# the-lay/voltools

Hardware: AMD Instinct MI355X
Metric: Mvoxels/s, 512^3 f32 filt_bspline StaticVolume transform (resident source, device output) (higher is better)
Workload: dtype f32; 1 GPU; 512^3 float32 filt_bspline, StaticVolume resident in HBM, rotate((0,i,0)) rzxz sweep, output= device buffer; lds_bytes=34816, kernel=8, resident_bytes=1660944384, angles=i

## Files before the change

voltools_amd/csrc/vt_api.hip:

```cpp
#include "vt_internal.h"
#include "vt_device.h"
#include "vt_host.h"

#include <atomic>
#include <cmath>
#include <cstdarg>
#include <cstdio>
#include <cstdlib>
#include <chrono>
#include <cstring>
#include <mutex>
#include <new>
#include <unordered_map>
#include <vector>

#include <unistd.h>

using namespace vt;

namespace vt_guard {
constexpr size_t kGuard = (size_t)1 << 20;
struct Entry { void* base; size_t bytes; };
static std::mutex mu;
static std::unordered_map<void*, Entry> live;
// ... 804 lines not shown
                VT_HIP(hipMalloc(&v->d_tplan, need));
                v->tplan_bytes = need;
                v->tplan_epoch = 0;
            }
            if (v->tplan_epoch == 0 || v->tplan_epoch == 0xffffffffu) {
                VT_HIP(hipMemsetAsync(v->d_tplan, 0, v->tplan_bytes, v->stream));
                v->tplan_epoch = 0;
            }
            q.tplan = v->d_tplan;
            q.tplan_epoch = ++v->tplan_epoch;
        }
        VT_HIP(launch_affine_quad(plan.cfg, v->interp, srcq, d_out, q, plan.grid, plan.lds_bytes, v->stream));
#ifdef VT_LEGACY
    } else if (plan.kind == 5) {
        float* const srcp = copy_ptr(v, kCopyP0 + ori.quad_idx);
        if (!srcp) return fail(VT_EINVAL, "internal: plane-pair copy missing");
        VT_HIP(launch_affine_zpair(plan.cfg, v->interp, srcp, d_out, p, plan.grid, plan.lds_bytes, v->stream));
#endif
    } else if (plan.kind == 9 || plan.kind == 6) {
        if (!v->d_queue) {
            VT_HIP(hipMalloc(reinterpret_cast<void**>(&v->d_queue), 9 * 128));
            VT_HIP(hipMemsetAsync(v->d_queue, 0, 9 * 128, v->stream));
        }
        if (plan.kind == 9) {
#ifdef VT_EXPERIMENTS
            static const int exp_lds = std::getenv("VT_EXP_BLOCK_LDS") ? std::atoi(std::getenv("VT_EXP_BLOCK_LDS")) : 0;
            static const int exp_grid = std::getenv("VT_EXP_BLOCK_GRID") ? std::atoi(std::getenv("VT_EXP_BLOCK_GRID")) : 0;
            VT_HIP(launch_affine_block(plan.cfg, plan.th, v->interp, ori.src_plain, d_out, v->d_zeros, v->d_queue, p, plan.geo, exp_grid > 0 ? exp_grid : plan.grid,
                                       std::max(plan.lds_bytes, exp_lds), v->stream));
#else
            VT_HIP(launch_affine_block(plan.cfg, plan.th, v->interp, ori.src_plain, d_out, v->d_zeros, v->d_queue, p, plan.geo, plan.grid, plan.lds_bytes, v->stream));
#endif
        }
        else if (!is_cubic(v->interp) && v->tune.span != 0)
            VT_HIP(launch_affine_span(plan.cfg, ori.src_plain, d_out, v->d_zeros, v->d_queue, p, plan.geo, plan.grid, plan.lds_bytes, v->stream));
        else
            VT_HIP(launch_affine_packed(plan.cfg, v->interp, ori.src_plain, d_out, v->d_zeros, v->d_queue, p, plan.geo, plan.grid, plan.lds_bytes, v->stream));
#ifdef VT_LEGACY
    } else if (plan.kind == 4) {
        VT_HIP(launch_affine_march(plan.cfg, v->interp, ori.src_plain, d_out, p, plan.grid, plan.lds_bytes, v->stream));
#endif
    } else if (plan.kind == 10) {
        VT_HIP(launch_affine_rows(v->interp, plan.td, ori.src_plain, d_out, v->d_zeros, p, plan.lds_bytes, v->stream));
    } else if (plan.kind >= 2) {
        VT_HIP(launch_affine_tiled(plan.cfg, v->interp, plan.kind == 3, ori.src_plain, d_out, v->d_zeros, p, plan.grid, plan.lds_bytes, v->stream));
    } else {
        VT_HIP(launch_affine_direct(v->interp, v->d_src, d_out, p, v->stream));
    }
    note_launch(v, plan.kind >= 2 ? plan.kind : 1, plan, p, n_out);
    return 0;
}

int host_output_buffer(vt_volume* v, size_t n_elems, float** d_out)
{
// ... 1484 lines not shown
                                (size_t)v->W * sizeof(float), rows, hipMemcpyDeviceToDevice, v->stream));
    else
        VT_HIP(pin.copy2d(v->d_src + (size_t)first_plane * v->H * v->P, (size_t)v->P * sizeof(float), data, (size_t)v->W * sizeof(float), rows, true, v->stream));
    VT_HIP(hipStreamSynchronize(v->stream));
    return 0;
}

int vt_volume_finalize(vt_volume_t* v)
{
    if (!v) return fail(VT_EINVAL, "NULL handle");
    if (!v->deferred) return 0;
    int rc = use_device(v->dev);
    if (rc) return rc;
    return finalize_resident(v, v->lo_interior);
}

int vt_volume_destroy(vt_volume_t* v)
{
    if (!v) return 0;
    hipSetDevice(v->dev);
    if (v->stream) hipStreamSynchronize(v->stream);
    if (v->d_src) cached_free(v->dev, v->d_src, v->src_bytes);
    if (v->d_queue) hipFree(v->d_queue);
    if (v->d_tplan) hipFree(v->d_tplan);
    {
        LazyCopies::Released rel;
        v->lazy.release_all(rel);
        for (void* b : rel.bufs) hipFree(b);
    }
    if (v->d_scratch_out) cached_free(v->dev, v->d_scratch_out, v->scratch_elems * sizeof(float));
    if (v->d_proj_tmp) hipFree(v->d_proj_tmp);
    if (v->d_proj_part) cached_free(v->dev, v->d_proj_part, v->proj_part_bytes);
    if (v->d_batch_m) hipFree(v->d_batch_m);
    if (v->proj) { vt_volume_destroy(v->proj); v->proj = nullptr; }
    if (v->ev0) recycle_event(v->dev, v->ev0);
    if (v->ev1) recycle_event(v->dev, v->ev1);
    if (v->evc0) (void)hipEventDestroy(v->evc0);
    if (v->evc1) (void)hipEventDestroy(v->evc1);
    if (v->stream && v->owns_stream) recycle_stream(v->dev, v->stream);
    delete v;
    return 0;
}

int vt_volume_release_copies(vt_volume_t* v, uint64_t* freed_bytes)
{
    if (!v) return fail(VT_EINVAL, "NULL argument");
// ... 314 lines not shown
```

voltools_amd/csrc/vt_device.h:

```cpp
#pragma once
#include "vt_internal.h"

namespace vt {


__host__ __device__ __forceinline__ void bspline_weights(float f, float& w0, float& w1, float& w2, float& w3)
{
    const float one_frac = 1.0f - f;
    const float squared = f * f;
    const float one_sqd = one_frac * one_frac;
    w0 = (1.0f / 6.0f) * one_sqd * one_frac;
    w1 = (2.0f / 3.0f) - 0.5f * squared * (2.0f - f);
    w2 = (2.0f / 3.0f) - 0.5f * one_sqd * (2.0f - one_frac);
    w3 = (1.0f / 6.0f) * squared * f;
}

__host__ __device__ __forceinline__ float bspline_fn(float t)
{
    t = fabsf(t);
    const float a = 2.0f - t;
    return (t < 1.0f) ? ((2.0f / 3.0f) - 0.5f * t * t * a) : ((t < 2.0f) ? (a * a * a * (1.0f / 6.0f)) : 0.0f);
}

template <bool SIMPLE>
// ... 12 lines not shown

__device__ __forceinline__ int wave_scan_add(int x)
{
    x += __builtin_amdgcn_update_dpp(0, x, 0x111, 0xf, 0xf, false);
    x += __builtin_amdgcn_update_dpp(0, x, 0x112, 0xf, 0xf, false);
    x += __builtin_amdgcn_update_dpp(0, x, 0x114, 0xf, 0xf, false);
    x += __builtin_amdgcn_update_dpp(0, x, 0x118, 0xf, 0xf, false);
    x += __builtin_amdgcn_update_dpp(0, x, 0x142, 0xa, 0xf, false);
    x += __builtin_amdgcn_update_dpp(0, x, 0x143, 0xc, 0xf, false);
    return x;
}
__device__ __forceinline__ int wave_scan_max(int x)
{
    x = max(x, __builtin_amdgcn_update_dpp(-1, x, 0x111, 0xf, 0xf, false));
    x = max(x, __builtin_amdgcn_update_dpp(-1, x, 0x112, 0xf, 0xf, false));
    x = max(x, __builtin_amdgcn_update_dpp(-1, x, 0x114, 0xf, 0xf, false));
    x = max(x, __builtin_amdgcn_update_dpp(-1, x, 0x118, 0xf, 0xf, false));
    x = max(x, __builtin_amdgcn_update_dpp(-1, x, 0x142, 0xa, 0xf, false));
    x = max(x, __builtin_amdgcn_update_dpp(-1, x, 0x143, 0xc, 0xf, false));
    return x;
}
__device__ __forceinline__ int wave_shift_up1(int x, int first) { return __builtin_amdgcn_update_dpp(first, x, 0x138, 0xf, 0xf, false); }

__device__ __forceinline__ int xcd_contiguous(int b, int n)
{
    const int xcd = b & 7, q = n >> 3, r = n & 7;
    const int start = (xcd < r) ? xcd * (q + 1) : r * (q + 1) + (xcd - r) * q;
    return start + (b >> 3);
}


__device__ __forceinline__ void march_tile(const AffineParams& p, int t, int& th_i, int& tw_i, int& chunk)
{
    const int per_layer = p.nTh * p.nTw;
    chunk = t / per_layer;
    const int u = t - chunk * per_layer;
    if (p.blk_h > 0) {
        const int col_tiles = p.nTh * p.blk_w;
        const int bc = u / col_tiles;
        const int wc = min(p.blk_w, p.nTw - bc * p.blk_w);
        const int u1 = u - bc * col_tiles;
        const int blk_tiles = p.blk_h * wc;
        const int br = u1 / blk_tiles;
        const int u2 = u1 - br * blk_tiles;
        const int r = u2 / wc;
        th_i = br * p.blk_h + r;
        tw_i = bc * p.blk_w + (u2 - r * wc);
    } else if (p.flags & (1 << 24)) {
        tw_i = u / p.nTh;
        th_i = u - tw_i * p.nTh;
    } else {
        th_i = u / p.nTw;
        tw_i = u - th_i * p.nTw;
    }
}

__host__ __device__ __forceinline__ int blocked_tile_count(int nTd, int nTh, int nTw)
{
    return ((nTd + 3) >> 2) * ((nTh + 3) >> 2) * ((nTw + 3) >> 2) * 64;
}
__device__ __forceinline__ bool blocked_tile(int t, int nTd, int nTh, int nTw, int& td, int& th, int& tw)
{
    const int nSh = (nTh + 3) >> 2, nSw = (nTw + 3) >> 2;
    const int sb = t >> 6, l = t & 63;
    const int sw = sb % nSw, s2 = sb / nSw;
    const int sh = s2 % nSh, sd = s2 / nSh;
    td = sd * 4 + (l >> 4);
    th = sh * 4 + ((l >> 2) & 3);
    tw = sw * 4 + (l & 3);
    return td < nTd && th < nTh && tw < nTw;
}

struct Fx { int hi; unsigned lo; };

constexpr double kBoxMargin = 0x1p-24;

__device__ __forceinline__ Fx to_fx(double x)
{
    const double fl = floor(x);
    Fx r;
    r.hi = (int)fl;
    r.lo = (unsigned)((x - fl) * 4294967296.0);
    return r;
}

__device__ __forceinline__ void fx_step(Fx& c, int inc_hi, unsigned inc_lo)
{
    const unsigned lo = c.lo + inc_lo;
    c.hi += inc_hi + (lo < c.lo ? 1 : 0);
    c.lo = lo;
}

__device__ __forceinline__ float fx_frac(const Fx& c) { return (float)c.lo * 0x1p-32f; }
// ... 189 lines not shown
```

voltools_amd/csrc/vt_host.h:

```cpp
#pragma once
#include "vt_internal.h"
#include "vt_resident.h"

#include <algorithm>
#include <cstdlib>
#include <vector>

struct Tuning {
    int tile = -1;
    int la = 0;
    int march_box = -1;
    int lxpad = -1;
    int dch = 0;
    int blk_h = -1, blk_w = -1;
    bool plain_tile_order = false;
    int rswap_wfast = -1;
    bool exp_nostore = false;
    bool exp_noload = false;
    bool exp_nolds = false;
    bool exp_noloop = false;
    bool exp_stamps = false;
    bool exp_notiles = false;
    bool exp_static = false;
    int quad_rows = -2;
// ... 2 lines not shown
    bool test_fail_copy = false;
    int quad_perm = 1;
    bool no_proj_cache = false;
    int quad_pingpong = 1;
    int quad_zid = 1;
    int reorient = 4;
    int rows_pd = 8;
    int no_fused_relayout = 0;
    int rows_db = 0;
    int rows = 1;
    int quad_zfir = 1;
    int zid_dch = 0;
    int quad_nt = -1;
    bool no_block = false;
    int block_rs = -1;
    bool block_linear = false;
    bool block_no_trim = false;
    int block_min = 240;
    int block_pad = -1;
    double max_resident_gb = 0.0;
    int span = 1;
    int span_pipe = 0;
    int block_th = 8;
    int64_t dot_part_cap = 64ll << 20;
    void read()
    {
        auto num = [](const char* name, int dflt) { const char* e = std::getenv(name); return e ? std::atoi(e) : dflt; };
        tile = num("VT_TILE", -1);
#ifdef VT_LEGACY
        la = num("VT_LA", 0);
        march_box = num("VT_MARCH_BOX", -1);
        if (march_box > 1) march_box = 1;
        lxpad = num("VT_LXPAD", -1);
#endif
        dch = std::max(0, num("VT_DCH", 0));
        blk_h = num("VT_BLK_H", -1);
        blk_w = num("VT_BLK_W", -1);
        plain_tile_order = num("VT_TILE_ORDER", 1) == 0;
        rswap_wfast = num("VT_RSWAP_WFAST", -1);
#ifdef VT_EXPERIMENTS
        exp_nostore = std::getenv("VT_EXP_NOSTORE") != nullptr;
        exp_noload = std::getenv("VT_EXP_NOLOAD") != nullptr;
        exp_nolds = std::getenv("VT_EXP_NOLDS") != nullptr;
        exp_noloop = std::getenv("VT_EXP_NOLOOP") != nullptr;
        exp_static = std::getenv("VT_EXP_STATIC") != nullptr;
        exp_notiles = std::getenv("VT_EXP_NOTILES") != nullptr;
// ... 2 lines not shown
        quad_nt = num("VT_QUAD_NT", -1);
#ifdef VT_LEGACY
        test_fail_copy = std::getenv("VT_TEST_FAIL_COPY") != nullptr;
        quad_perm = num("VT_QUAD_PERM", 1);
        quad_zid = num("VT_QUAD_ZID", 1);
        quad_grid2d = num("VT_QUAD_GRID2D", 1);
#endif
        quad_pingpong = num("VT_QUAD_PINGPONG", 1);
        quad_zfir = num("VT_QUAD_ZFIR", 1);
        rows = num("VT_ROWS", 1);
        rows_pd = num("VT_ROWS_PD", 8);
        rows_db = num("VT_ROWS_DB", 0);
        no_fused_relayout = num("VT_NO_FUSED_RELAYOUT", 0);
        reorient = num("VT_REORIENT", 4);
        no_proj_cache = std::getenv("VT_NO_PROJ_CACHE") != nullptr;
        zid_dch = num("VT_ZID_DCH", 0);
        quad_reverse = num("VT_QUAD_REVERSE", -1);
        quad_rows = num("VT_QUAD_ROWS", -2);
        no_block = std::getenv("VT_NO_BLOCK_KERNEL") != nullptr;
        block_rs = num("VT_BLOCK_RS", -1);
        block_linear = std::getenv("VT_BLOCK_LINEAR") != nullptr;
        block_pad = num("VT_BLOCK_PAD", -1);
        block_th = num("VT_BLOCK_TH", 8) == 16 ? 16 : 8;
        span_pipe = num("VT_SPAN_PIPE", 0);
        span = num("VT_SPAN", 1);
        { const char* e = std::getenv("VT_MAX_RESIDENT_GB"); max_resident_gb = e ? std::atof(e) : 0.0; }
        block_min = std::max(1, num("VT_BLOCK_MIN", 240));
        block_no_trim = std::getenv("VT_BLOCK_NO_TRIM") != nullptr;
        { const char* e = std::getenv("VT_DOT_PART_CAP"); if (e && std::atoll(e) > 0) dot_part_cap = std::min<int64_t>(std::atoll(e), 64ll << 20); }
    }
};


struct vt_volume {
    unsigned launch_no = 0;
    int dev = 0;
    int interp = 0;
    int D = 0, H = 0, W = 0;
    int oD = 0, oH = 0, oW = 0;
    int64_t plane0 = 0;
    int64_t gD = 0;
    int64_t out_plane0 = 0;
    int P = 0;
    float* d_src = nullptr;
    size_t src_bytes = 0;
    float* d_zeros = nullptr;
    int Pr = 0;
    int Px = 0;
    int reorient_asked[3] = {0, 0, 0};
    vt::LazyCopies lazy;
    float copies_ms = 0.f;
    int copies_built = 0, copies_evicted = 0;
    hipEvent_t evc0 = nullptr, evc1 = nullptr;
    int* d_queue = nullptr;
    void* d_tplan = nullptr;
    size_t tplan_bytes = 0;
    uint32_t tplan_epoch = 0;
    float* d_scratch_out = nullptr;
    double* d_batch_m = nullptr;
    std::vector<double> h_batch_m;
    size_t batch_m_cap = 0;
    float* d_proj_tmp = nullptr;
    size_t proj_tmp_elems = 0;
    double* d_proj_part = nullptr;
    size_t proj_part_bytes = 0;
    vt_volume* proj = nullptr;
    bool proj_sum_valid = false;
    double proj_sum_m3 = 0.0;
    int proj_sum_oD = 0;
    int64_t proj_sum_oplane0 = 0;
    int edge_pad = 0;
    bool stack = false;
    bool owns_stream = true;
    bool deferred = false;
    bool lo_interior = false;
    size_t scratch_elems = 0;
    hipStream_t stream = nullptr;
// ... 20 lines not shown
```

voltools_amd/csrc/vt_internal.h:

```cpp
#pragma once
#include <hip/hip_runtime.h>
#include <math.h>
#include <stdint.h>
#include "../../include/voltools_hip.h"

namespace vt {

constexpr float kPole   = -0x1.126148p-2f;
constexpr float kLambda =  0x1.7ffffep+2f;
constexpr float kAntiInit = 0x1.b0cb1ap-3f;

struct AffineParams {
    double m[12];
    double neg[3];
    double pos[3];
    double vlo[3];
    double vhi[3];
    int32_t inc_hi[3];
    uint32_t inc_lo[3];
    int32_t sD, sH, sW;
    int32_t sP;
    int32_t oD, oH, oW;
    int32_t nTd, nTh, nTw;
    int32_t Lz, Ly, Lx;
// ... 161 lines not shown
hipError_t launch_relayout_swap01(const float* src, float* dst, int D, int H, int P, hipStream_t stream);
int quad_max_it();
int quad_config_count();
void quad_config(int idx, int* th, int* tw, int* nt);
int quad_tile_plan_granules(int cfg);
int quad_tile_plan_lds(int cfg);
int quad_blocks_per_cu(int cfg, int interp, int lds_bytes, bool zid = false);
hipError_t init_quad_kernels();
hipError_t launch_relayout_zquad(const float* src, float* dst, int D, int H, int W, int P, int Pq, hipStream_t stream);
hipError_t launch_relayout_xfir(const float* src, float* dst, int D, int H, int W, int P, bool simple, hipStream_t stream);
hipError_t init_rows_kernels();
void rows_tile(int* ph, int* run);
hipError_t launch_affine_rows(int interp, int pd, const float* src, float* out, const float* zeros16, const AffineParams& p, int lds_bytes, hipStream_t stream);
hipError_t launch_relayout_zquad_fir(const float* src, float* dst, int D, int H, int W, int P, int Pq, bool simple, hipStream_t stream);
hipError_t launch_relayout_zquad_swap12(const float* src, float* dst, int D, int H, int W, int P, int Pq, bool fir, bool simple, hipStream_t stream);
hipError_t launch_affine_quad(int cfg, int interp, const float* srcq, float* out, const AffineParams& p,
                              int grid, int lds_bytes, hipStream_t stream);
int block_rs_count();
int block_rs(int idx);
int block_rs_order(int th, const int** order);
int block_max_vectors(int th);
void block_tile(int th, int* td, int* tw);
hipError_t init_block_kernels();
hipError_t launch_affine_block(int rs_idx, int th, int interp, const float* src, float* out, const float* zeros16, int* queue,
                               const AffineParams& p, const PackGeom& geo, int grid, int lds_bytes, hipStream_t stream);
int packed_config_count();
void packed_config(int idx, int* td, int* th, int* tw);
int packed_rows_max();
int packed_vectors_max();
hipError_t init_packed_kernels();
hipError_t launch_affine_packed(int cfg, int interp, const float* src, float* out, const float* zeros16, int* queue,
                                const AffineParams& p, const PackGeom& geo, int grid, int lds_bytes, hipStream_t stream);
int span_config_count();
void span_config(int idx, int* td, int* th, int* tw);
int span_rows_max();
bool span_config_pipelined(int idx);
int span_vectors_max();
hipError_t init_span_kernels();
hipError_t launch_affine_span(int cfg, const float* src, float* out, const float* zeros16, int* queue,
                              const AffineParams& p, const PackGeom& geo, int grid, int lds_bytes, hipStream_t stream);
int march_rows_max();
int march_max_it();
int interp_kind(int interp);
hipError_t init_march_kernels();
hipError_t launch_affine_march(int cfg, int interp, const float* src, float* out, const AffineParams& p,
                               int grid, int lds_bytes, hipStream_t stream);
hipError_t launch_affine_direct(int interp, const float* src, float* out, const AffineParams& p,
// ... 94 lines not shown
```

voltools_amd/csrc/vt_kernels_block.hip:

```cpp
#include "vt_internal.h"
#include "vt_device.h"

#include <algorithm>
#include <type_traits>

namespace vt {

typedef float v2f __attribute__((ext_vector_type(2)));

constexpr int kBlkTD = 8, kBlkTW = 16;
constexpr int block_max_it(int th) { return th == 16 ? 20 : 13; }

template <int OFF>
__device__ __forceinline__ void lds_read_b64(v2f& r, unsigned a)
{
    asm volatile("ds_read_b64 %0, %1 offset:%2" : "=v"(r) : "v"(a), "n"(OFF));
}

__device__ __forceinline__ v2f pk_fma(v2f a, float w, v2f c) { return __builtin_elementwise_fma(a, (v2f)(w), c); }

__device__ __forceinline__ void bspline_weights_pk(float f, v2f& w30, v2f& w12)
{
    const v2f fg = {f, 1.0f - f};
    const v2f sq = fg * fg;
// ... 66 lines not shown
                         (unsigned)gx < (unsigned)p.sP;
        const float* g = inb ? src + (((int64_t)gz * p.sH + gy) * p.sP + gx) : zeros16;
        __builtin_amdgcn_global_load_lds((const __attribute__((address_space(1))) void*)g,
                                         (__attribute__((address_space(3))) void*)(lds + 4 * vb), 16, 0, 0);
    }
}

template <int RS, int MAXIT>
__device__ __forceinline__ void stage_block_checked(float* lds, const float* __restrict__ src, const float* __restrict__ zeros16,
                                                    const AffineParams& p, const int (&o)[3], const int (&voff)[MAXIT], int total, int psv, int tid)
{
    constexpr int nvx = RS / 4;
    const int wave_first = __builtin_amdgcn_readfirstlane(tid & ~63);
    const char* const origin = reinterpret_cast<const char*>(src + (((int64_t)o[0] * p.sH + o[1]) * p.sP + o[2]));
#pragma unroll
    for (int k = 0; k < MAXIT; ++k) {
        if (k * 256 + wave_first < total) {
            int v = k * 256 + tid;
            asm volatile("" : "+v"(v));
            const int z = (int)__umulhi((unsigned)v, p.psv_magic), rem = v - z * psv;
            const int y = rem / nvx, cx = rem - y * nvx;
            const int gz = o[0] + z, gy = o[1] + y, gx = o[2] + 4 * cx;
            const bool inb = (unsigned)gz < (unsigned)p.sD && (unsigned)gy < (unsigned)p.sH && (unsigned)gx < (unsigned)p.sP;
            const float* g = inb ? reinterpret_cast<const float*>(origin + voff[k]) : zeros16;
            if (voff[k] != 0 || v == 0)
                __builtin_amdgcn_global_load_lds((const __attribute__((address_space(1))) void*)g,
                                                 (__attribute__((address_space(3))) void*)(lds + 4 * (k * 256 + wave_first)), 16, 0, 0);
        }
    }
}

template <int KIND, int RS, int TH>
__device__ __forceinline__ void affine_block_body(const float* __restrict__ src, float* __restrict__ out, const float* __restrict__ zeros16,
                                                  int* __restrict__ queue, const AffineParams& p, const PackGeom& geo)
{
    constexpr bool CUBIC = KIND != 0;
    constexpr int HALO = CUBIC ? 1 : 0;
    constexpr int TD = kBlkTD, TW = kBlkTW;
    constexpr int NS = TH == 16 ? 8 : 4;
    constexpr int kBlkMaxIt = block_max_it(TH);
    constexpr bool PIN = TH == 16;
    constexpr int nvx = RS / 4;
    extern __shared__ __attribute__((aligned(16))) float lds[];

    const int tid = threadIdx.x, lane = tid & 63, wv = tid >> 6;
    const int wave_first = __builtin_amdgcn_readfirstlane(tid & ~63);
    const int vd = lane >> 4, vh = 4 * (wv >> 1) + ((lane >> 2) & 3), vw = 4 * (wv & 1) + (lane & 3);
    constexpr int sd[8] = {0, 0, TH == 16 ? 0 : 4, TH == 16 ? 0 : 4, 4, 4, 4, 4};
    constexpr int sh[8] = {0, 0, TH == 16 ? 8 : 0, TH == 16 ? 8 : 0, 8, 8, 0, 0};
    constexpr int sw[8] = {0, 8, 8, 0, 0, 8, 8, 0};
    constexpr int which[7] = {0, TH == 16 ? 1 : 3, 2, 3, 0, 4, 2};

    const int Lz = p.Lz, Ly = p.Ly, ps = p.Lps;
    const int psv = ps >> 2;
    const int total = Lz * psv;
    const int nvx_used = p.Lx_used >> 2;
    const int row_b = p.sP * 4;
    const int plane_b = p.sH * row_b;

    int voff[kBlkMaxIt];
#pragma unroll
    for (int k = 0; k < kBlkMaxIt; ++k) {
        const int v = k * 256 + tid;
        const int z = (int)__umulhi((unsigned)v, p.psv_magic), rem = v - z * psv;
        const int y = rem / nvx, cx = rem - y * nvx;
        bool used = v < total && y < Ly && cx < nvx_used;
        if (used && (p.flags & (1 << 25))) {
            int mn, mx;
            used = packed_row_span(geo, z, y, &mn, &mx);
            used = used && cx >= (mn >> 2) && cx <= (mx >> 2);
        }
        voff[k] = used ? z * plane_b + y * row_b + 16 * cx : 0;
    }

    const bool keep = (p.flags & VT_KEEP_OUTSIDE) != 0;
    const int64_t ostride = (int64_t)p.oH * p.oW;
    const int obase = (int)((vd * ostride + (int64_t)vh * p.oW + vw) * 4);
    const int ostep_d = (int)(4 * ostride * 4), ostep_h = (int)(8 * (int64_t)p.oW * 4);
    const unsigned ps4 = 4u * (unsigned)ps;
    const unsigned lds_base = lds_byte_address(lds);
    int inc_hi[5][3];
    unsigned inc_lo[5][3];
#pragma unroll
    for (int k = 0; k < 5; ++k)
#pragma unroll
        for (int r = 0; r < 3; ++r) {
            inc_hi[k][r] = p.binc_hi[k][r];
            inc_lo[k][r] = p.binc_lo[k][r];
            if (PIN || k == 0 || k == 2 || k == 3) asm volatile("" : "+v"(inc_hi[k][r]), "+v"(inc_lo[k][r]));
        }
    double gm[12], gneg[3], gpos[3], gvlo[3], gvhi[3];
    double mp[3][3];
    const int oc0 = p.ord[0], oc1 = p.ord[1], oc2 = p.ord[2];
    auto load_consts = [&](const auto& kp_) {
        const auto* const kp = &kp_;
// ... 20 lines not shown
        }
    }
    double toff[3];
#pragma unroll
    for (int r = 0; r < 3; ++r) toff[r] = fma(p.m[4 * r], (double)vd, fma(p.m[4 * r + 1], (double)vh, p.m[4 * r + 2] * (double)vw));
    auto inside_canonical = [&](int d, int h, int w) {
        const double x0 = (double)(oc0 == 0 ? d : (oc0 == 1 ? h : w));
        const double x1 = (double)(oc1 == 0 ? d : (oc1 == 1 ? h : w));
        const double x2 = (double)(oc2 == 0 ? d : (oc2 == 1 ? h : w));
        bool in = true;
#pragma unroll
        for (int r = 0; r < 3; ++r) {
            const double sc = fma(mp[r][0], x0, fma(mp[r][1], x1, fma(mp[r][2], x2, gm[4 * r + 3])));
            in = in && (sc >= gvlo[r]) && (sc < gvhi[r]);
        }
        return in;
    };
#ifdef VT_EXPERIMENTS
    const bool no_stores = (p.flags & (1 << 21)) != 0, no_loads = (p.flags & (1 << 22)) != 0, no_lds = (p.flags & (1 << 26)) != 0;
#else
    constexpr bool no_stores = false, no_loads = false, no_lds = false;
#endif

    int* const ctrl = reinterpret_cast<int*>(lds + (p.lds_cap >> 2));
    const int nids = blocked_tile_count(p.nTd, p.nTh, p.nTw);
    const int nSh = (p.nTh + 3) >> 2, nSw = (p.nTw + 3) >> 2;
    const int xcd = blockIdx.x & 7, per = ((nids >> 6) + 7) / 8 * 64;
    const int id0 = xcd * per, id_cnt = max(0, min(per, nids - id0));
    int* const counter = queue + 32 * xcd;
    const int chunk = p.dch;
    int nxt = 0;
    if (tid == 0) nxt = atomicAdd(counter, chunk);
    int cur = 0, left = 0;
    for (;;) {
        if (left == 0) {
            if (tid == 0) ctrl[0] = nxt;
            __syncthreads();
            cur = ctrl[0];
            left = chunk;
            __syncthreads();
            if (cur >= id_cnt) break;
            if (tid == 0) nxt = atomicAdd(counter, chunk);
        }
        const int id = id0 + cur;
        ++cur; --left;
        if (cur > id_cnt) continue;
        int td_i, th_i, tw_i;
        const unsigned sbi = (unsigned)id >> 6, l6 = (unsigned)id & 63u;
        const unsigned s2 = nSw == 1 ? sbi : __umulhi(sbi, p.nTw_magic), sbw = sbi - s2 * (unsigned)nSw;
        const unsigned sbd = nSh == 1 ? s2 : __umulhi(s2, p.nTh_magic), sbh = s2 - sbd * (unsigned)nSh;
        td_i = (int)(sbd * 4 + (l6 >> 4)); th_i = (int)(sbh * 4 + ((l6 >> 2) & 3)); tw_i = (int)(sbw * 4 + (l6 & 3));
        const bool tile_ok = td_i < p.nTd && th_i < p.nTh && tw_i < p.nTw;
        if (!tile_ok) continue;
        if constexpr (!PIN) {
            typedef const __attribute__((address_space(4))) char* KArg;
            KArg ka = (KArg)__builtin_amdgcn_kernarg_segment_ptr();
            asm volatile("" : "+s"(ka));
            load_consts(*(const __attribute__((address_space(4))) AffineParams*)(ka + 32));
        }
        const int d0 = td_i * TD, h0 = th_i * TH, w0 = tw_i * TW;

        double base[3], lo[3], hi[3];
        bool any_valid = true, all_valid = true;
#pragma unroll
        for (int r = 0; r < 3; ++r) {
            base[r] = fma(gm[4 * r], (double)d0, fma(gm[4 * r + 1], (double)h0, fma(gm[4 * r + 2], (double)w0, gm[4 * r + 3])));
            lo[r] = base[r] + gneg[r];
            hi[r] = base[r] + gpos[r];
            any_valid = any_valid && (hi[r] >= gvlo[r] - kTileMargin) && (lo[r] < gvhi[r] + kTileMargin);
            all_valid = all_valid && (lo[r] >= gvlo[r] + kTileMargin) && (hi[r] < gvhi[r] - kTileMargin);
        }
        float* const otile = out + ((int64_t)d0 * ostride + (int64_t)h0 * p.oW + w0);
        __amdgpu_buffer_rsrc_t orsrc = __builtin_amdgcn_make_buffer_rsrc(reinterpret_cast<char*>(otile), 0, 0x7fffffff, 0x00020000);
        const bool whole = (d0 + TD <= p.oD) && (h0 + TH <= p.oH) && (w0 + TW <= p.oW);

        if (!any_valid) {
            if (!keep) {
#pragma unroll
                for (int s = 0; s < NS; ++s) {
                    const int d = d0 + vd + sd[s], h = h0 + vh + sh[s], w = w0 + vw + sw[s];
                    if (whole || (d < p.oD && h < p.oH && w < p.oW))
                        __builtin_amdgcn_raw_buffer_store_b32(0u, orsrc, obase, (sd[s] >> 2) * ostep_d + (sh[s] >> 3) * ostep_h + 4 * sw[s], 0);
                }
            }
            continue;
        }

        int o[3];
#pragma unroll
        for (int r = 0; r < 3; ++r) o[r] = (int)floor(lo[r]) - HALO;
        o[2] &= ~3;
        const bool box_inside = o[0] >= 0 && o[1] >= 0 && o[2] >= 0 && o[0] + Lz <= p.sD && o[1] + Ly <= p.sH && o[2] + p.Lx_used <= p.sP;

        __syncthreads();
        if (no_loads) {
        } else if (box_inside) {
            __amdgpu_buffer_rsrc_t rsrc = __builtin_amdgcn_make_buffer_rsrc(
                const_cast<char*>(reinterpret_cast<const char*>(src + (((int64_t)o[0] * p.sH + o[1]) * p.sP + o[2]))), 0, 0x7fffffff, 0x00020000);
            char* dst = reinterpret_cast<char*>(lds) + 16 * wave_first;
#pragma unroll
            for (int k = 0; k < kBlkMaxIt; ++k)
                if (k * 256 + wave_first < total)
                    __builtin_amdgcn_raw_ptr_buffer_load_lds(rsrc, (__attribute__((address_space(3))) void*)(dst + 4096 * k), 16, voff[k], 0, 0, 0);
        } else {
            if constexpr (TH == 16) stage_block_checked_box<RS>(lds, src, zeros16, p, o, total, psv, nvx_used, tid);
            else stage_block_checked<RS, kBlkMaxIt>(lds, src, zeros16, p, o, voff, total, psv, tid);
        }
        Fx c[3];
#pragma unroll
        for (int r = 0; r < 3; ++r) c[r] = to_fx((base[r] - (double)o[r]) + toff[r]);
        asm volatile("s_waitcnt vmcnt(0)" ::: "memory");
        __syncthreads();

        unsigned inmask = (1u << NS) - 1u, zmask = 0u;
        if (!(all_valid && whole)) {
            inmask = 0u;
            if constexpr (!PIN) {
                typedef const __attribute__((address_space(4))) char* KArg;
                KArg ka = (KArg)__builtin_amdgcn_kernarg_segment_ptr();
                asm volatile("" : "+s"(ka));
                load_chain(*(const __attribute__((address_space(4))) AffineParams*)(ka + 32));
// ... 25 lines not shown
                const float x00 = fmaf(fx, a001 - a000, a000);
                const float x01 = fmaf(fx, a011 - a010, a010);
                const float x10 = fmaf(fx, a101 - a100, a100);
                const float x11 = fmaf(fx, a111 - a110, a110);
                const float y0 = fmaf(fy, x01 - x00, x00);
                const float y1 = fmaf(fy, x11 - x10, x10);
                val = fmaf(fz, y1 - y0, y0);
            }
            asm volatile("" : "+v"(val));
            const int soff = (sd[s] >> 2) * ostep_d + (sh[s] >> 3) * ostep_h + 4 * sw[s];
            if (no_stores) {
                if (val == 123.456f) __builtin_amdgcn_raw_buffer_store_b32(__builtin_bit_cast(unsigned, val), orsrc, obase, soff, 0);
            } else if ((inmask >> s) & 1u) {
                __builtin_amdgcn_raw_buffer_store_b32(__builtin_bit_cast(unsigned, val), orsrc, obase, soff, 0);
            } else if ((zmask >> s) & 1u) {
                __builtin_amdgcn_raw_buffer_store_b32(0u, orsrc, obase, soff, 0);
            }
            if (s < NS - 1) {
#pragma unroll
                for (int r = 0; r < 3; ++r) fx_step(c[r], inc_hi[which[s]][r], inc_lo[which[s]][r]);
            }
            asm volatile("" : "+v"(c[0].hi), "+v"(c[0].lo), "+v"(c[1].hi), "+v"(c[1].lo), "+v"(c[2].hi), "+v"(c[2].lo));
        }
    }
    if (tid == 0) {
        __threadfence();
        if (atomicAdd(&queue[256], 1) == (int)gridDim.x - 1) {
#pragma unroll
            for (int i = 0; i < 9; ++i) queue[32 * i] = 0;
        }
    }
}

template <int KIND, int RS>
__global__ __launch_bounds__(256, 2) void affine_block(const float* __restrict__ src, float* __restrict__ out, const float* __restrict__ zeros16,
                                                        int* __restrict__ queue, const AffineParams p, const PackGeom geo)
{
    affine_block_body<KIND, RS, 16>(src, out, zeros16, queue, p, geo);
}
template <int KIND, int RS>
__global__ __launch_bounds__(256, 4) void affine_block_half(const float* __restrict__ src, float* __restrict__ out, const float* __restrict__ zeros16,
                                                             int* __restrict__ queue, const AffineParams p, const PackGeom geo)
{
    affine_block_body<KIND, RS, 8>(src, out, zeros16, queue, p, geo);
}

typedef void (*block_fn)(const float*, float*, const float*, int*, const AffineParams, const PackGeom);

static const int kBlkRS[] = {28, 36, 32, 12, 20, 16, 24};
static const int kOrder16[] = {0, 1, 2};
static const int kOrder8[] = {3, 4, 0, 1, 5, 6, 2};
int block_rs_count() { return (int)(sizeof(kBlkRS) / sizeof(kBlkRS[0])); }
int block_rs(int idx) { return kBlkRS[idx]; }
int block_rs_order(int th, const int** order) { *order = th == 16 ? kOrder16 : kOrder8; return th == 16 ? 3 : 7; }
int block_max_vectors(int th) { return 256 * block_max_it(th); }
void block_tile(int th, int* td, int* tw) { (void)th; *td = kBlkTD; *tw = kBlkTW; }

template <int RS, int TH>
static block_fn pick_block_kind(int kind)
{
    if constexpr (TH == 16) {
        switch (kind) {
            case 0: return affine_block<0, RS>;
            case 1: return affine_block<1, RS>;
            default: return affine_block<2, RS>;
        }
    } else {
        switch (kind) {
            case 0: return affine_block_half<0, RS>;
            case 1: return affine_block_half<1, RS>;
            default: return affine_block_half<2, RS>;
        }
    }
}

static block_fn block_entry(int rs_idx, int kind, int th)
{
    if (th == 16) return rs_idx == 0 ? pick_block_kind<28, 16>(kind) : (rs_idx == 1 ? pick_block_kind<36, 16>(kind) : pick_block_kind<32, 16>(kind));
    switch (rs_idx) {
        case 0: return pick_block_kind<28, 8>(kind);
        case 1: return pick_block_kind<36, 8>(kind);
        case 2: return pick_block_kind<32, 8>(kind);
        case 3: return pick_block_kind<12, 8>(kind);
        case 4: return pick_block_kind<20, 8>(kind);
        case 5: return pick_block_kind<16, 8>(kind);
        default: return pick_block_kind<24, 8>(kind);
    }
}

hipError_t init_block_kernels()
{
    for (int th = 8; th <= 16; th += 8)
        for (int rs = 0; rs < (th == 16 ? 3 : block_rs_count()); ++rs)
            for (int kind = 0; kind < 3; ++kind) {
                hipError_t e = hipFuncSetAttribute(reinterpret_cast<const void*>(block_entry(rs, kind, th)),
                                                   hipFuncAttributeMaxDynamicSharedMemorySize, 160 * 1024);
                if (e != hipSuccess) return e;
            }
    return hipSuccess;
}

hipError_t launch_affine_block(int rs_idx, int th, int interp, const float* src, float* out, const float* zeros16, int* queue,
                               const AffineParams& p, const PackGeom& geo, int grid, int lds_bytes, hipStream_t stream)
{
    hipLaunchKernelGGL(block_entry(rs_idx, interp_kind(interp), th), dim3(grid), dim3(256), lds_bytes, stream, src, out, zeros16, queue, p, geo);
    return hipGetLastError();
}

}
```

voltools_amd/csrc/vt_plan.hip:

```cpp
#include "vt_host.h"
#include "vt_device.h"

#include <cmath>
#include <cstring>

namespace vt {
namespace {

struct PlanCtx {
    const vt_volume* v;
    const double* m;
    int flags;
    AffineParams* p;
    TilePlan* plan;
    bool cubic;
    bool zsep;
    int halo2;
};

#ifdef VT_LEGACY
int64_t round_aware_chunks(int64_t oD, int g, int64_t inplane, int64_t resident, int64_t n0, int extra, int min_dch, int64_t n_floor)
{
    if (resident <= 0 || inplane > resident || inplane * n0 >= 16 * resident) return n0;
    auto cost = [&](int64_t n) {
// ... 681 lines not shown
    double tot = 0;
    for (int b = 0; b < 4; ++b) {
        int words[32], n = 0;
        for (int l = 0; l < 32; ++l) {
            const int t[3] = {lm == 0 ? (l >> 4) : 0, lm == 0 ? ((l >> 2) & 3) : (l >> 4), lm == 0 ? (l & 3) : (l & 15)};
            int f[3];
            for (int r = 0; r < 3; ++r)
                f[r] = (int)std::floor(kBase[b][r] + 24.0 + m[4 * r] * t[0] + m[4 * r + 1] * t[1] + m[4 * r + 2] * t[2]);
            const int a = f[0] * PS + f[1] * RS + (cubic ? (((f[2] - 1) & ~1) >> 1) * 2 : f[2]);
            const int word = cubic ? (a >> 1) : a;
            bool seen = false;
            for (int i = 0; i < n; ++i) seen = seen || words[i] == word;
            if (!seen) words[n++] = word;
        }
        int cnt[32] = {0}, worst = 0;
        for (int i = 0; i < n; ++i) worst = std::max(worst, ++cnt[((words[i] % 32) + 32) % 32]);
        tot += worst;
    }
    return tot / 4.0;
}

bool plan_block_th(PlanCtx& c, int th);

bool plan_block(PlanCtx& c)
{
    if (c.v->tune.block_th == 8 && plan_block_th(c, 8)) return true;
    return plan_block_th(c, 16);
}

bool plan_block_th(PlanCtx& c, int th)
{
    const vt_volume* v = c.v;
    const double* m = c.m;
    AffineParams* p = c.p;
    TilePlan* plan = c.plan;
    if ((c.flags & (VT_NO_BLOCK | VT_NO_PACKED | VT_FORCE_PACKED)) || v->tune.no_block) return false;
    if (c.zsep) return false;
    if (!c.cubic && !v->tune.block_linear) return false;
    if (!(c.flags & VT_FORCE_TILED) && (int64_t)v->oD * v->oH * v->oW < (int64_t)v->tune.block_min * v->tune.block_min * v->tune.block_min) return false;
    int T[3];
    T[1] = th;
    block_tile(th, &T[0], &T[2]);
    int L[3];
    for (int r = 0; r < 3; ++r) {
        double ext = 0;
        for (int k = 0; k < 3; ++k) ext += std::fabs(m[4 * r + k]) * (T[k] - 1);
// ... 65 lines not shown
    const double mul[5] = {8.0, 8.0, -8.0, 4.0, -8.0};
    const int neg_of[5] = {-1, -1, 0, -1, 1};
    for (int s = 0; s < 5; ++s)
        for (int r = 0; r < 3; ++r) {
            if (neg_of[s] >= 0) {
                const uint64_t fwd = ((uint64_t)(uint32_t)p->binc_hi[neg_of[s]][r] << 32) | p->binc_lo[neg_of[s]][r];
                const uint64_t back = 0 - fwd;
                p->binc_hi[s][r] = (int32_t)(uint32_t)(back >> 32); p->binc_lo[s][r] = (uint32_t)back;
                continue;
            }
            const double step = m[4 * r + col[s]] * mul[s];
            const double fl = std::floor(step);
            double lo = std::floor((step - fl) * 4294967296.0 + 0.5);
            int32_t hi = (int32_t)fl;
            if (lo >= 4294967296.0) { lo = 0; hi += 1; }
            p->binc_hi[s][r] = hi; p->binc_lo[s][r] = (uint32_t)lo;
        }
    plan->blocks_per_cu = (int)std::min<int64_t>(th == 16 ? 2 : 4, (160 * 1024) / lds_bytes);
    const int64_t ids = blocked_tile_count(p->nTd, p->nTh, p->nTw);
    int64_t grid = std::min<int64_t>((int64_t)v->cu_count * plan->blocks_per_cu, ids);
    grid = std::max<int64_t>(8, (grid + 7) / 8 * 8);
    p->dch = (int)std::max<int64_t>(1, std::min<int64_t>(4, ids / (grid * 8)));
    plan->grid = (int)grid;
    return true;
}

bool plan_general(PlanCtx& c)
{
    double box_bpv = 1e300;
    const bool have_box = pick_box_tile(c, &box_bpv);
    if (plan_packed(c, have_box, box_bpv)) return true;
    if (!have_box) return false;
    const double* mm = c.m;
    const double det = mm[0] * (mm[5] * mm[10] - mm[6] * mm[9]) - mm[1] * (mm[4] * mm[10] - mm[6] * mm[8]) + mm[2] * (mm[4] * mm[9] - mm[5] * mm[8]);
    if (c.plan->kind == 2 && !(c.flags & VT_FORCE_TILED) && c.v->tune.tile < 0 && std::fabs(det) >= 9.0 &&
        (c.plan->lds_bytes > 80 * 1024 || (!c.cubic && box_bpv > 43.0))) {
        c.plan->kind = 1; c.plan->cfg = -1; c.plan->td = c.plan->th = c.plan->tw = 0; c.plan->lds_bytes = 0; c.plan->grid = 0;
        return true;
    }
    if (!finish_box(c)) { c.plan->kind = 1; }
    return true;
}

typedef bool (*plan_fn)(PlanCtx&);
struct Family { const char* name; plan_fn plan; };
const Family kFamilies[] = {
// ... 137 lines not shown
```

Measured before the change: 706,300 Mvoxels/s.

## Launch block kernel as static grid with cached per-thread offset table

Adds a grid-launched form of the half-height block kernel. Each workgroup maps its block index straight to a fixed brick of tiles along W, replacing the persistent atomic work queue. The per-thread vector offsets are precomputed once into a device table, keyed on the transform's linear part and geometry, and reused across calls. The first tile skips a barrier, and the tile origins are made wave-uniform for the buffer descriptor. This removes atomics, queue-control barriers and per-block offset arithmetic, at the cost of many more, short-lived workgroups and the loss of dynamic load balancing.

```diff
diff --git a/voltools_amd/csrc/vt_api.hip b/voltools_amd/csrc/vt_api.hip
--- a/voltools_amd/csrc/vt_api.hip
+++ b/voltools_amd/csrc/vt_api.hip
@@ -850,14 +850,31 @@
             VT_HIP(hipMalloc(reinterpret_cast<void**>(&v->d_queue), 9 * 128));
             VT_HIP(hipMemsetAsync(v->d_queue, 0, 9 * 128, v->stream));
         }
-        if (plan.kind == 9) {
+        if (plan.kind == 9 && (p.flags & (1 << 23))) {
+            vt_volume::BlockTabKey key = {};
+            for (int r = 0; r < 3; ++r)
+                for (int k = 0; k < 3; ++k) key.lin[3 * r + k] = p.m[4 * r + k];
+            key.rs = p.Lx; key.Lz = p.Lz; key.Ly = p.Ly; key.Lps = p.Lps; key.Lx_used = p.Lx_used; key.trim = (p.flags >> 25) & 1;
+            key.sH = p.sH; key.sP = p.sP;
+            if (!v->d_block_tab) {
+                VT_HIP(hipMalloc(reinterpret_cast<void**>(&v->d_block_tab), (size_t)block_table_bytes()));
+                v->block_tab_valid = false;
+            }
+            if (!v->block_tab_valid || std::memcmp(&key, &v->block_tab_key, sizeof(key)) != 0) {
+                v->block_tab_valid = false;
+                VT_HIP(launch_block_voff_table(v->d_block_tab, p, plan.geo, v->stream));
+                v->block_tab_key = key;
+                v->block_tab_valid = true;
+            }
+            VT_HIP(launch_affine_block(plan.cfg, plan.th, v->interp, true, ori.src_plain, d_out, v->d_zeros, v->d_block_tab, p, plan.geo, plan.grid, plan.lds_bytes, v->stream));
+        } else if (plan.kind == 9) {
 #ifdef VT_EXPERIMENTS
             static const int exp_lds = std::getenv("VT_EXP_BLOCK_LDS") ? std::atoi(std::getenv("VT_EXP_BLOCK_LDS")) : 0;
             static const int exp_grid = std::getenv("VT_EXP_BLOCK_GRID") ? std::atoi(std::getenv("VT_EXP_BLOCK_GRID")) : 0;
-            VT_HIP(launch_affine_block(plan.cfg, plan.th, v->interp, ori.src_plain, d_out, v->d_zeros, v->d_queue, p, plan.geo, exp_grid > 0 ? exp_grid : plan.grid,
+            VT_HIP(launch_affine_block(plan.cfg, plan.th, v->interp, false, ori.src_plain, d_out, v->d_zeros, v->d_queue, p, plan.geo, exp_grid > 0 ? exp_grid : plan.grid,
                                        std::max(plan.lds_bytes, exp_lds), v->stream));
 #else
-            VT_HIP(launch_affine_block(plan.cfg, plan.th, v->interp, ori.src_plain, d_out, v->d_zeros, v->d_queue, p, plan.geo, plan.grid, plan.lds_bytes, v->stream));
+            VT_HIP(launch_affine_block(plan.cfg, plan.th, v->interp, false, ori.src_plain, d_out, v->d_zeros, v->d_queue, p, plan.geo, plan.grid, plan.lds_bytes, v->stream));
 #endif
         }
         else if (!is_cubic(v->interp) && v->tune.span != 0)
@@ -2388,6 +2405,7 @@
     if (v->stream) hipStreamSynchronize(v->stream);
     if (v->d_src) cached_free(v->dev, v->d_src, v->src_bytes);
     if (v->d_queue) hipFree(v->d_queue);
+    if (v->d_block_tab) hipFree(v->d_block_tab);
     if (v->d_tplan) hipFree(v->d_tplan);
     {
         LazyCopies::Released rel;
diff --git a/voltools_amd/csrc/vt_device.h b/voltools_amd/csrc/vt_device.h
--- a/voltools_amd/csrc/vt_device.h
+++ b/voltools_amd/csrc/vt_device.h
@@ -58,7 +58,7 @@
 }
 __device__ __forceinline__ int wave_shift_up1(int x, int first) { return __builtin_amdgcn_update_dpp(first, x, 0x138, 0xf, 0xf, false); }
 
-__device__ __forceinline__ int xcd_contiguous(int b, int n)
+__host__ __device__ __forceinline__ int xcd_contiguous(int b, int n)
 {
     const int xcd = b & 7, q = n >> 3, r = n & 7;
     const int start = (xcd < r) ? xcd * (q + 1) : r * (q + 1) + (xcd - r) * q;
@@ -95,7 +95,7 @@
 {
     return ((nTd + 3) >> 2) * ((nTh + 3) >> 2) * ((nTw + 3) >> 2) * 64;
 }
-__device__ __forceinline__ bool blocked_tile(int t, int nTd, int nTh, int nTw, int& td, int& th, int& tw)
+__host__ __device__ __forceinline__ bool blocked_tile(int t, int nTd, int nTh, int nTw, int& td, int& th, int& tw)
 {
     const int nSh = (nTh + 3) >> 2, nSw = (nTw + 3) >> 2;
     const int sb = t >> 6, l = t & 63;
@@ -105,6 +105,22 @@
     th = sh * 4 + ((l >> 2) & 3);
     tw = sw * 4 + (l & 3);
     return td < nTd && th < nTh && tw < nTw;
+}
+__host__ __device__ __forceinline__ unsigned block_magic(int n) { return (unsigned)((1ULL << 32) / (unsigned long long)n + 1ULL); }
+__host__ __device__ __forceinline__ bool blocked_tile_magic(int t, int nTd, int nTh, int nTw, unsigned magic_w, unsigned magic_h,
+                                                            int& td, int& th, int& tw)
+{
+    const unsigned nSh = (unsigned)(nTh + 3) >> 2, nSw = (unsigned)(nTw + 3) >> 2;
+    const unsigned sbi = (unsigned)t >> 6, l6 = (unsigned)t & 63u;
+    const unsigned s2 = nSw == 1 ? sbi : (unsigned)(((unsigned long long)sbi * magic_w) >> 32), sbw = sbi - s2 * nSw;
+    const unsigned sbd = nSh == 1 ? s2 : (unsigned)(((unsigned long long)s2 * magic_h) >> 32), sbh = s2 - sbd * nSh;
+    td = (int)(sbd * 4 + (l6 >> 4)); th = (int)(sbh * 4 + ((l6 >> 2) & 3)); tw = (int)(sbw * 4 + (l6 & 3));
+    return td < nTd && th < nTh && tw < nTw;
+}
+__host__ __device__ __forceinline__ bool block_grid_tile(int b, int n, int brick, int nTd, int nTh, int nTw, unsigned magic_w, unsigned magic_h,
+                                                         int& td, int& th, int& tw)
+{
+    return blocked_tile_magic(xcd_contiguous(b, n) * brick, nTd, nTh, nTw, magic_w, magic_h, td, th, tw);
 }
 
 struct Fx { int hi; unsigned lo; };
diff --git a/voltools_amd/csrc/vt_host.h b/voltools_amd/csrc/vt_host.h
--- a/voltools_amd/csrc/vt_host.h
+++ b/voltools_amd/csrc/vt_host.h
@@ -48,6 +48,8 @@
     int span = 1;
     int span_pipe = 0;
     int block_th = 8;
+    int block_grid = -1;
+    int block_brick = 0;
     int64_t dot_part_cap = 64ll << 20;
     void read()
     {
@@ -96,6 +98,9 @@
         block_linear = std::getenv("VT_BLOCK_LINEAR") != nullptr;
         block_pad = num("VT_BLOCK_PAD", -1);
         block_th = num("VT_BLOCK_TH", 8) == 16 ? 16 : 8;
+        block_grid = std::getenv("VT_BLOCK_GRID") ? (num("VT_BLOCK_GRID", 0) != 0 ? 1 : 0) : -1;
+        block_brick = num("VT_BLOCK_BRICK", 0);
+        if (block_brick != 1 && block_brick != 2 && block_brick != 4) block_brick = 0;
         span_pipe = num("VT_SPAN_PIPE", 0);
         span = num("VT_SPAN", 1);
         { const char* e = std::getenv("VT_MAX_RESIDENT_GB"); max_resident_gb = e ? std::atof(e) : 0.0; }
@@ -127,6 +132,9 @@
     int copies_built = 0, copies_evicted = 0;
     hipEvent_t evc0 = nullptr, evc1 = nullptr;
     int* d_queue = nullptr;
+    int* d_block_tab = nullptr;
+    struct BlockTabKey { double lin[9]; int32_t rs, Lz, Ly, Lps, Lx_used, trim, sH, sP; } block_tab_key = {};
+    bool block_tab_valid = false;
     void* d_tplan = nullptr;
     size_t tplan_bytes = 0;
     uint32_t tplan_epoch = 0;
diff --git a/voltools_amd/csrc/vt_internal.h b/voltools_amd/csrc/vt_internal.h
--- a/voltools_amd/csrc/vt_internal.h
+++ b/voltools_amd/csrc/vt_internal.h
@@ -207,7 +207,9 @@
 int block_max_vectors(int th);
 void block_tile(int th, int* td, int* tw);
 hipError_t init_block_kernels();
-hipError_t launch_affine_block(int rs_idx, int th, int interp, const float* src, float* out, const float* zeros16, int* queue,
+int block_table_bytes();
+hipError_t launch_block_voff_table(int* table, const AffineParams& p, const PackGeom& geo, hipStream_t stream);
+hipError_t launch_affine_block(int rs_idx, int th, int interp, bool grid_form, const float* src, float* out, const float* zeros16, int* queue,
                                const AffineParams& p, const PackGeom& geo, int grid, int lds_bytes, hipStream_t stream);
 int packed_config_count();
 void packed_config(int idx, int* td, int* th, int* tw);
diff --git a/voltools_amd/csrc/vt_kernels_block.hip b/voltools_amd/csrc/vt_kernels_block.hip
--- a/voltools_amd/csrc/vt_kernels_block.hip
+++ b/voltools_amd/csrc/vt_kernels_block.hip
@@ -112,7 +112,7 @@
             const int y = rem / nvx, cx = rem - y * nvx;
             const int gz = o[0] + z, gy = o[1] + y, gx = o[2] + 4 * cx;
             const bool inb = (unsigned)gz < (unsigned)p.sD && (unsigned)gy < (unsigned)p.sH && (unsigned)gx < (unsigned)p.sP;
-            const float* g = inb ? reinterpret_cast<const float*>(origin + voff[k]) : zeros16;
+            const float* g = inb ? reinterpret_cast<const float*>(origin + (unsigned)voff[k]) : zeros16;
             if (voff[k] != 0 || v == 0)
                 __builtin_amdgcn_global_load_lds((const __attribute__((address_space(1))) void*)g,
                                                  (__attribute__((address_space(3))) void*)(lds + 4 * (k * 256 + wave_first)), 16, 0, 0);
@@ -120,10 +120,33 @@
     }
 }
 
-template <int KIND, int RS, int TH>
+__device__ __forceinline__ int block_voff(const AffineParams& p, const PackGeom& geo, int v, int nvx)
+{
+    const int psv = p.Lps >> 2;
+    const int row_b = p.sP * 4;
+    const int plane_b = p.sH * row_b;
+    const int z = (int)__umulhi((unsigned)v, p.psv_magic), rem = v - z * psv;
+    const int y = rem / nvx, cx = rem - y * nvx;
+    bool used = v < p.Lz * psv && y < p.Ly && cx < (p.Lx_used >> 2);
+    if (used && (p.flags & (1 << 25))) {
+        int mn, mx;
+        used = packed_row_span(geo, z, y, &mn, &mx);
+        used = used && cx >= (mn >> 2) && cx <= (mx >> 2);
+    }
+    return used ? z * plane_b + y * row_b + 16 * cx : 0;
+}
+
+__global__ __launch_bounds__(256) void block_voff_table(int* __restrict__ tab, const AffineParams p, const PackGeom geo)
+{
+    const int nvx = p.Lx >> 2;
+    for (int k = 0; k < block_max_it(8); ++k) tab[k * 256 + threadIdx.x] = block_voff(p, geo, k * 256 + (int)threadIdx.x, nvx);
+}
+
+template <int KIND, int RS, int TH, bool GRID>
 __device__ __forceinline__ void affine_block_body(const float* __restrict__ src, float* __restrict__ out, const float* __restrict__ zeros16,
                                                   int* __restrict__ queue, const AffineParams& p, const PackGeom& geo)
 {
+    static_assert(!GRID || TH == 8, "the grid-launched form serves the half-height tile");
     constexpr bool CUBIC = KIND != 0;
     constexpr int HALO = CUBIC ? 1 : 0;
     constexpr int TD = kBlkTD, TW = kBlkTW;
@@ -145,22 +168,17 @@
     const int psv = ps >> 2;
     const int total = Lz * psv;
     const int nvx_used = p.Lx_used >> 2;
-    const int row_b = p.sP * 4;
-    const int plane_b = p.sH * row_b;
+
+    int g_td = 0, g_th = 0, g_tw = 0;
+    if constexpr (GRID) {
+        if (!block_grid_tile((int)blockIdx.x, (int)gridDim.x, p.dch, p.nTd, p.nTh, p.nTw, p.nTw_magic, p.nTh_magic, g_td, g_th, g_tw)) return;
+    }
 
     int voff[kBlkMaxIt];
 #pragma unroll
     for (int k = 0; k < kBlkMaxIt; ++k) {
-        const int v = k * 256 + tid;
-        const int z = (int)__umulhi((unsigned)v, p.psv_magic), rem = v - z * psv;
-        const int y = rem / nvx, cx = rem - y * nvx;
-        bool used = v < total && y < Ly && cx < nvx_used;
-        if (used && (p.flags & (1 << 25))) {
-            int mn, mx;
-            used = packed_row_span(geo, z, y, &mn, &mx);
-            used = used && cx >= (mn >> 2) && cx <= (mx >> 2);
-        }
-        voff[k] = used ? z * plane_b + y * row_b + 16 * cx : 0;
+        if constexpr (GRID) voff[k] = queue[k * 256 + tid];
+        else voff[k] = block_voff(p, geo, k * 256 + tid, nvx);
     }
 
     const bool keep = (p.flags & VT_KEEP_OUTSIDE) != 0;
@@ -227,36 +245,7 @@
     constexpr bool no_stores = false, no_loads = false, no_lds = false;
 #endif
 
-    int* const ctrl = reinterpret_cast<int*>(lds + (p.lds_cap >> 2));
-    const int nids = blocked_tile_count(p.nTd, p.nTh, p.nTw);
-    const int nSh = (p.nTh + 3) >> 2, nSw = (p.nTw + 3) >> 2;
-    const int xcd = blockIdx.x & 7, per = ((nids >> 6) + 7) / 8 * 64;
-    const int id0 = xcd * per, id_cnt = max(0, min(per, nids - id0));
-    int* const counter = queue + 32 * xcd;
-    const int chunk = p.dch;
-    int nxt = 0;
-    if (tid == 0) nxt = atomicAdd(counter, chunk);
-    int cur = 0, left = 0;
-    for (;;) {
-        if (left == 0) {
-            if (tid == 0) ctrl[0] = nxt;
-            __syncthreads();
-            cur = ctrl[0];
-            left = chunk;
-            __syncthreads();
-            if (cur >= id_cnt) break;
-            if (tid == 0) nxt = atomicAdd(counter, chunk);
-        }
-        const int id = id0 + cur;
-        ++cur; --left;
-        if (cur > id_cnt) continue;
-        int td_i, th_i, tw_i;
-        const unsigned sbi = (unsigned)id >> 6, l6 = (unsigned)id & 63u;
-        const unsigned s2 = nSw == 1 ? sbi : __umulhi(sbi, p.nTw_magic), sbw = sbi - s2 * (unsigned)nSw;
-        const unsigned sbd = nSh == 1 ? s2 : __umulhi(s2, p.nTh_magic), sbh = s2 - sbd * (unsigned)nSh;
-        td_i = (int)(sbd * 4 + (l6 >> 4)); th_i = (int)(sbh * 4 + ((l6 >> 2) & 3)); tw_i = (int)(sbw * 4 + (l6 & 3));
-        const bool tile_ok = td_i < p.nTd && th_i < p.nTh && tw_i < p.nTw;
-        if (!tile_ok) continue;
+    auto do_tile = [&](int td_i, int th_i, int tw_i, bool fresh) __attribute__((always_inline)) {
         if constexpr (!PIN) {
             typedef const __attribute__((address_space(4))) char* KArg;
             KArg ka = (KArg)__builtin_amdgcn_kernarg_segment_ptr();
@@ -288,7 +277,7 @@
                         __builtin_amdgcn_raw_buffer_store_b32(0u, orsrc, obase, (sd[s] >> 2) * ostep_d + (sh[s] >> 3) * ostep_h + 4 * sw[s], 0);
                 }
             }
-            continue;
+            return;
         }
 
         int o[3];
@@ -297,11 +286,12 @@
         o[2] &= ~3;
         const bool box_inside = o[0] >= 0 && o[1] >= 0 && o[2] >= 0 && o[0] + Lz <= p.sD && o[1] + Ly <= p.sH && o[2] + p.Lx_used <= p.sP;
 
-        __syncthreads();
+        if (!fresh) __syncthreads();
         if (no_loads) {
         } else if (box_inside) {
+            const int os0 = __builtin_amdgcn_readfirstlane(o[0]), os1 = __builtin_amdgcn_readfirstlane(o[1]), os2 = __builtin_amdgcn_readfirstlane(o[2]);
             __amdgpu_buffer_rsrc_t rsrc = __builtin_amdgcn_make_buffer_rsrc(
-                const_cast<char*>(reinterpret_cast<const char*>(src + (((int64_t)o[0] * p.sH + o[1]) * p.sP + o[2]))), 0, 0x7fffffff, 0x00020000);
+                const_cast<char*>(reinterpret_cast<const char*>(src + (((int64_t)os0 * p.sH + os1) * p.sP + os2))), 0, 0x7fffffff, 0x00020000);
             char* dst = reinterpret_cast<char*>(lds) + 16 * wave_first;
 #pragma unroll
             for (int k = 0; k < kBlkMaxIt; ++k)
@@ -373,6 +363,39 @@
             }
             asm volatile("" : "+v"(c[0].hi), "+v"(c[0].lo), "+v"(c[1].hi), "+v"(c[1].lo), "+v"(c[2].hi), "+v"(c[2].lo));
         }
+    };
+
+    if constexpr (GRID) {
+        const int last = min(p.dch, p.nTw - g_tw);
+        for (int j = 0; j < last; ++j) do_tile(g_td, g_th, g_tw + j, j == 0);
+        return;
+    }
+
+    int* const ctrl = reinterpret_cast<int*>(lds + (p.lds_cap >> 2));
+    const int nids = blocked_tile_count(p.nTd, p.nTh, p.nTw);
+    const int xcd = blockIdx.x & 7, per = ((nids >> 6) + 7) / 8 * 64;
+    const int id0 = xcd * per, id_cnt = max(0, min(per, nids - id0));
+    int* const counter = queue + 32 * xcd;
+    const int chunk = p.dch;
+    int nxt = 0;
+    if (tid == 0) nxt = atomicAdd(counter, chunk);
+    int cur = 0, left = 0;
+    for (;;) {
+        if (left == 0) {
+            if (tid == 0) ctrl[0] = nxt;
+            __syncthreads();
+            cur = ctrl[0];
+            left = chunk;
+            __syncthreads();
+            if (cur >= id_cnt) break;
+            if (tid == 0) nxt = atomicAdd(counter, chunk);
+        }
+        const int id = id0 + cur;
+        ++cur; --left;
+        if (cur > id_cnt) continue;
+        int td_i, th_i, tw_i;
+        if (!blocked_tile_magic(id, p.nTd, p.nTh, p.nTw, p.nTw_magic, p.nTh_magic, td_i, th_i, tw_i)) continue;
+        do_tile(td_i, th_i, tw_i, false);
     }
     if (tid == 0) {
         __threadfence();
@@ -387,13 +410,19 @@
 __global__ __launch_bounds__(256, 2) void affine_block(const float* __restrict__ src, float* __restrict__ out, const float* __restrict__ zeros16,
                                                         int* __restrict__ queue, const AffineParams p, const PackGeom geo)
 {
-    affine_block_body<KIND, RS, 16>(src, out, zeros16, queue, p, geo);
+    affine_block_body<KIND, RS, 16, false>(src, out, zeros16, queue, p, geo);
 }
 template <int KIND, int RS>
 __global__ __launch_bounds__(256, 4) void affine_block_half(const float* __restrict__ src, float* __restrict__ out, const float* __restrict__ zeros16,
                                                              int* __restrict__ queue, const AffineParams p, const PackGeom geo)
 {
-    affine_block_body<KIND, RS, 8>(src, out, zeros16, queue, p, geo);
+    affine_block_body<KIND, RS, 8, false>(src, out, zeros16, queue, p, geo);
+}
+template <int KIND, int RS>
+__global__ __launch_bounds__(256, 4) void affine_block_grid(const float* __restrict__ src, float* __restrict__ out, const float* __restrict__ zeros16,
+                                                             int* __restrict__ voff_table, const AffineParams p, const PackGeom geo)
+{
+    affine_block_body<KIND, RS, 8, true>(src, out, zeros16, voff_table, p, geo);
 }
 
 typedef void (*block_fn)(const float*, float*, const float*, int*, const AffineParams, const PackGeom);
@@ -407,7 +436,7 @@
 int block_max_vectors(int th) { return 256 * block_max_it(th); }
 void block_tile(int th, int* td, int* tw) { (void)th; *td = kBlkTD; *tw = kBlkTW; }
 
-template <int RS, int TH>
+template <int RS, int TH, bool GRID>
 static block_fn pick_block_kind(int kind)
 {
     if constexpr (TH == 16) {
@@ -416,6 +445,12 @@
             case 1: return affine_block<1, RS>;
             default: return affine_block<2, RS>;
         }
+    } else if constexpr (GRID) {
+        switch (kind) {
+            case 0: return affine_block_grid<0, RS>;
+            case 1: return affine_block_grid<1, RS>;
+            default: return affine_block_grid<2, RS>;
+        }
     } else {
         switch (kind) {
             case 0: return affine_block_half<0, RS>;
@@ -425,36 +460,52 @@
     }
 }
 
-static block_fn block_entry(int rs_idx, int kind, int th)
-{
-    if (th == 16) return rs_idx == 0 ? pick_block_kind<28, 16>(kind) : (rs_idx == 1 ? pick_block_kind<36, 16>(kind) : pick_block_kind<32, 16>(kind));
+template <bool GRID>
+static block_fn block_entry_half(int rs_idx, int kind)
+{
     switch (rs_idx) {
-        case 0: return pick_block_kind<28, 8>(kind);
-        case 1: return pick_block_kind<36, 8>(kind);
-        case 2: return pick_block_kind<32, 8>(kind);
-        case 3: return pick_block_kind<12, 8>(kind);
-        case 4: return pick_block_kind<20, 8>(kind);
-        case 5: return pick_block_kind<16, 8>(kind);
-        default: return pick_block_kind<24, 8>(kind);
-    }
+        case 0: return pick_block_kind<28, 8, GRID>(kind);
+        case 1: return pick_block_kind<36, 8, GRID>(kind);
+        case 2: return pick_block_kind<32, 8, GRID>(kind);
+        case 3: return pick_block_kind<12, 8, GRID>(kind);
+        case 4: return pick_block_kind<20, 8, GRID>(kind);
+        case 5: return pick_block_kind<16, 8, GRID>(kind);
+        default: return pick_block_kind<24, 8, GRID>(kind);
+    }
+}
+
+static block_fn block_entry(int rs_idx, int kind, int th, bool grid_form)
+{
+    if (th == 16) return rs_idx == 0 ? pick_block_kind<28, 16, false>(kind) : (rs_idx == 1 ? pick_block_kind<36, 16, false>(kind) : pick_block_kind<32, 16, false>(kind));
+    return grid_form ? block_entry_half<true>(rs_idx, kind) : block_entry_half<false>(rs_idx, kind);
 }
 
 hipError_t init_block_kernels()
 {
-    for (int th = 8; th <= 16; th += 8)
-        for (int rs = 0; rs < (th == 16 ? 3 : block_rs_count()); ++rs)
-            for (int kind = 0; kind < 3; ++kind) {
-                hipError_t e = hipFuncSetAttribute(reinterpret_cast<const void*>(block_entry(rs, kind, th)),
-                                                   hipFuncAttributeMaxDynamicSharedMemorySize, 160 * 1024);
-                if (e != hipSuccess) return e;
-            }
+    for (int form = 0; form < 2; ++form)
+        for (int th = 8; th <= 16; th += 8)
+            for (int rs = 0; rs < (th == 16 ? 3 : block_rs_count()); ++rs)
+                for (int kind = 0; kind < 3; ++kind) {
+                    if (form == 1 && th == 16) continue;
+                    hipError_t e = hipFuncSetAttribute(reinterpret_cast<const void*>(block_entry(rs, kind, th, form == 1)),
+                                                       hipFuncAttributeMaxDynamicSharedMemorySize, 160 * 1024);
+                    if (e != hipSuccess) return e;
+                }
     return hipSuccess;
 }
 
-hipError_t launch_affine_block(int rs_idx, int th, int interp, const float* src, float* out, const float* zeros16, int* queue,
+int block_table_bytes() { return 256 * block_max_it(8) * (int)sizeof(int); }
+
+hipError_t launch_block_voff_table(int* table, const AffineParams& p, const PackGeom& geo, hipStream_t stream)
+{
+    hipLaunchKernelGGL(block_voff_table, dim3(1), dim3(256), 0, stream, table, p, geo);
+    return hipGetLastError();
+}
+
+hipError_t launch_affine_block(int rs_idx, int th, int interp, bool grid_form, const float* src, float* out, const float* zeros16, int* queue,
                                const AffineParams& p, const PackGeom& geo, int grid, int lds_bytes, hipStream_t stream)
 {
-    hipLaunchKernelGGL(block_entry(rs_idx, interp_kind(interp), th), dim3(grid), dim3(256), lds_bytes, stream, src, out, zeros16, queue, p, geo);
+    hipLaunchKernelGGL(block_entry(rs_idx, interp_kind(interp), th, grid_form), dim3(grid), dim3(256), lds_bytes, stream, src, out, zeros16, queue, p, geo);
     return hipGetLastError();
 }
 
diff --git a/voltools_amd/csrc/vt_plan.hip b/voltools_amd/csrc/vt_plan.hip
--- a/voltools_amd/csrc/vt_plan.hip
+++ b/voltools_amd/csrc/vt_plan.hip
@@ -727,6 +727,13 @@
 
 bool plan_block_th(PlanCtx& c, int th);
 
+constexpr int kBlockGridBrick = 2;
+constexpr int kBlockGridMaxEdge = 512;
+static bool block_grid_default(const vt_volume* v)
+{
+    return (int64_t)v->oD * v->oH * v->oW <= (int64_t)kBlockGridMaxEdge * kBlockGridMaxEdge * kBlockGridMaxEdge;
+}
+
 bool plan_block(PlanCtx& c)
 {
     if (c.v->tune.block_th == 8 && plan_block_th(c, 8)) return true;
@@ -838,6 +845,13 @@
     grid = std::max<int64_t>(8, (grid + 7) / 8 * 8);
     p->dch = (int)std::max<int64_t>(1, std::min<int64_t>(4, ids / (grid * 8)));
     plan->grid = (int)grid;
+    const bool grid_form = th == 8 && (v->tune.block_grid >= 0 ? v->tune.block_grid == 1 : block_grid_default(v));
+    if (grid_form) {
+        const int brick = v->tune.block_brick ? v->tune.block_brick : kBlockGridBrick;
+        p->flags |= (1 << 23);
+        p->dch = brick;
+        plan->grid = (int)(ids / brick);
+    }
     return true;
 }
 
```

Result: no change. 706,700 Mvoxels/s (median of 2 runs) (+0.0%).
